# sebasv/lp

Measured on NVIDIA B200. Metric: ipm_iterations_per_s, higher is better.
Workload: dtype f64

## Files before the change

### lp_b200/build.py

```python
from __future__ import annotations

import os
import subprocess
import sys
from concurrent.futures import ThreadPoolExecutor

HERE = os.path.dirname(os.path.abspath(__file__))
CSRC = os.path.join(HERE, "csrc")
LIBDIR = os.path.join(HERE, "_lib")
OBJDIR = os.path.join(LIBDIR, "obj")
LIB = os.path.join(LIBDIR, "liblpb200.so")
SOURCES = ["vec_kernels.cu", "dmma_gemm.cu", "cholesky.cu", "batched.cu", "presolve.cu", "lpb_api.cu"]
NVCC = os.environ.get("NVCC", "/usr/local/cuda/bin/nvcc")
FLAGS = ["-gencode", "arch=compute_100a,code=sm_100a", "-O3", "-std=c++17", "-lineinfo",
         "-Xcompiler", "-fPIC", "-Xcompiler", "-fvisibility=hidden"] + os.environ.get("LPB_EXTRA_NVCC_FLAGS", "").split()


def _deps():
    out = []
    for root in (CSRC, os.path.join(HERE, "..", "include")):
        for f in os.listdir(root):
            if f.endswith((".cu", ".cuh", ".hpp", ".h")):
                out.append(os.path.join(root, f))
    return out


def _stale(target, deps):
    if not os.path.exists(target):
        return True
    t = os.path.getmtime(target)
    return any(os.path.getmtime(d) > t for d in deps)


def build(force: bool = False, verbose: bool = True) -> str:
    os.makedirs(OBJDIR, exist_ok=True)
    deps = _deps()
    srcs = [s for s in SOURCES if os.path.exists(os.path.join(CSRC, s))]

    def compile_one(src):
        obj = os.path.join(OBJDIR, src.replace(".cu", ".o"))
        if force or _stale(obj, deps):
            cmd = [NVCC] + FLAGS + ["-c", os.path.join(CSRC, src), "-o", obj]
            if verbose:
                print(" ".join(cmd), flush=True)
            subprocess.check_call(cmd)
        return obj

    with ThreadPoolExecutor(max_workers=4) as ex:
        objs = list(ex.map(compile_one, srcs))
    if force or _stale(LIB, objs):
        cmd = [NVCC, "-shared", "-o", LIB] + objs + ["-lnccl", "-Xlinker", "-rpath=/usr/local/cuda/lib64"]
        if verbose:
            print(" ".join(cmd), flush=True)
        subprocess.check_call(cmd)
    return LIB


if __name__ == "__main__":
    print(build(force="--force" in sys.argv))
```

### lp_b200/csrc/common.cuh

```cuda
#pragma once
#include <cuda_runtime.h>
#include <cstdint>
#include <cstdio>
#include <cstring>
#include <mutex>

#include "../../include/lpb200.h"

namespace lpb {

void set_last_error(const char* fmt, ...);
const char* get_last_error();

#define LPB_CUDA(call)                                                                         \
  do {                                                                                         \
    cudaError_t e__ = (call);                                                                  \
    if (e__ != cudaSuccess) {                                                                  \
      ::lpb::set_last_error("%s:%d %s -> %s", __FILE__, __LINE__, #call, cudaGetErrorString(e__)); \
      return LPB_ERR_CUDA;                                                                     \
    }                                                                                          \
  } while (0)

#define LPB_TRY(call)              \
  do {                             \
    int rc__ = (call);             \
    if (rc__ != LPB_OK) return rc__; \
  } while (0)

constexpr int kNumSMs = 148;

constexpr int kMaxDevices = 64;
struct PerDeviceOnce {
  std::mutex mu;
  bool done[kMaxDevices] = {};
  template <class F>
  int run(F&& f) {
    int dev = 0;
    LPB_CUDA(cudaGetDevice(&dev));
    if (dev < 0 || dev >= kMaxDevices) return f(dev);
    std::lock_guard<std::mutex> g(mu);
    if (done[dev]) return LPB_OK;
    const int rc = f(dev);
    if (rc == LPB_OK) done[dev] = true;
    return rc;
  }
};

inline int64_t round_up(int64_t v, int64_t a) { return (v + a - 1) / a * a; }
inline int64_t ceil_div(int64_t a, int64_t b) { return (a + b - 1) / b; }

constexpr int kMaxRedVals = 8;
constexpr int kMaxRedBlocks = 1024;
enum RedOp : int { kRedSum = 0, kRedMin = 1 };

struct LaunchCtx {
  cudaStream_t stream = nullptr;
  int64_t launches = 0;
  double* red_partials = nullptr;
  double* red_out = nullptr;
  double* red_host = nullptr;
  unsigned long long* fault_dev = nullptr;
  double* gemv_partials = nullptr;
  int64_t gemv_partials_cap = 0;
  double* chol_ws = nullptr;
  int64_t chol_ws_cap = 0;
  int64_t ws_m = -1;
  int64_t linv_valid_m = -1;
  const double* linv_mat = nullptr;
  bool linv_full = false;
  int solve_epoch = 0;
  int solve_impl = 0;
  int sync_each_launch = 0;
  int syrk_flush_blocks = 32;
  int syrk_tail_split = 1;
  double* syrk_ws = nullptr;
  int64_t syrk_ws_cap = 0;
  int syrk_chain = 0;
  int potf2_impl = 0;
  int trsm_impl = 0, update_impl = 0;
  int solve_grid_cap = 0;
  void* nccl_comm = nullptr;
  int rank = 0, world = 1;
  int potrf_dist = 2;
  double* panel_buf = nullptr;
  int64_t panel_buf_cap = 0;
  int potrf_lookahead = 1;
  cudaStream_t side_stream = nullptr;
  cudaEvent_t ev_col[2] = {nullptr, nullptr}, ev_pan[2] = {nullptr, nullptr};
  bool launch_on_side = false;
  cudaEvent_t ev_dist[4] = {nullptr, nullptr, nullptr, nullptr};
  double* panel_slot[2] = {nullptr, nullptr};
  int64_t panel_slot_cap = 0;
  static constexpr int kMaxPeers = 8;
  double* ring_base = nullptr;
  int64_t ring_slot_doubles = 0;
  int ring_slots = 0;
  double* peer_base[kMaxPeers] = {};
  bool peer_mapped = false;
  bool peer_ready = false;
  uint32_t dist_epoch = 0;
  int update_grid_cap = 0;
  int* info_dev = nullptr;
  int* info_host = nullptr;
};

}
```

### lp_b200/csrc/kernels.hpp

```cpp
#pragma once
#include "common.cuh"

namespace lpb {

struct RedSpec {
  int nvals = 0;
  int nblocks[kMaxRedVals] = {0};
  int op[kMaxRedVals] = {0};
};
int reduce_finalize(LaunchCtx& lc, const RedSpec& spec);
int fetch_scalars(LaunchCtx& lc, int nvals);

int k_fill(LaunchCtx& lc, double* p, int64_t n, double v);
int k_copy(LaunchCtx& lc, double* dst, const double* src, int64_t n);
int k_dinv(LaunchCtx& lc, int64_t n, const double* x, const double* z, double* dinv);

int k_rhat(LaunchCtx& lc, int64_t n, int mode, double eta, double gm, double a2, double s, const double* x,
           const double* z, const double* rD, const double* dx, const double* dz, double* xs, double* r1);

int k_assemble_delta_n(LaunchCtx& lc, int64_t n, double d_tau, const double* u, const double* p, const double* xs,
                       const double* x, const double* z, double* dx, double* dz, int val_base, int* nblocks);
int k_assemble_delta_m(LaunchCtx& lc, int64_t m, double d_tau, const double* v, const double* q, double* dy);
int k_step(LaunchCtx& lc, int64_t n, double alpha, int clamp, double* x, const double* dx);
int k_extract_x(LaunchCtx& lc, int64_t n, double tau, const double* x, const double* c, double* xo, int val,
                int* nblocks);

int k_resid_p(LaunchCtx& lc, int64_t m, double tau, const double* b, const double* t, const double* y, double* rP,
              int val_base, int* nblocks);
int k_sym_fwd_rhs(LaunchCtx& lc, int64_t m, double eta, const double* rP, const double* b, const double* t0,
                  const double* t1, double* rhs0, double* rhs1, int with_pq);
int k_refine_rhs(LaunchCtx& lc, int64_t m, double eta, const double* rP, const double* b, const double* au,
                 const double* ap, double* rho0, double* rho1, int with_pq);
int k_add_inplace(LaunchCtx& lc, int64_t count, const double* x, double* y);
int k_dots_m(LaunchCtx& lc, int64_t m, const double* b, const double* v, const double* q, int with_pq, int val_base,
             int* nblocks);

int k_gemv_n(LaunchCtx& lc, int64_t m, int64_t n, const double* A, int64_t lda, const double* dinv, const double* w0,
             const double* w1, double* t0, double* t1, int nrhs);
int k_gemv_t_partials(LaunchCtx& lc, int64_t m, int64_t n, const double* A, int64_t lda, const double* v0,
                      const double* v1, int nrhs, int* nchunks);
struct TailCols {
  int64_t nd;
  const int* col_row;
  const double* col_val;
  const double* v0;
  const double* v1;
};
int k_gemv_t_raw(LaunchCtx& lc, int64_t n, int nchunks, int nrhs, double* out0, double* out1);
int k_resid_d(LaunchCtx& lc, int64_t n, int nchunks, double tau, const double* c, const double* z, const double* x,
              double* rD, int val_base, int* nblocks, const TailCols* tail = nullptr);
int k_sym_back(LaunchCtx& lc, int64_t n, int nchunks, int with_pq, const double* dinv, const double* r1,
               const double* c, double* u, double* p, int val_base, int* nblocks, const TailCols* tail = nullptr);

int k_syrk_dmma(LaunchCtx& lc, int64_t m, int64_t n, const double* A, int64_t lda, const double* d, double* Cmat,
                int64_t ldc);
int k_trailing_update_dmma(LaunchCtx& lc, int64_t m, double* Mat, int64_t ldm, int64_t k0, int64_t kb);
int k_trailing_update_part(LaunchCtx& lc, int64_t m, double* Mat, int64_t ldm, int64_t k0, int64_t kb, int tile0,
                           int single_col, int own_mod, int own_rem, const double* packed = nullptr,
                           int64_t packed_rows = 0);
int k_trsm_dmma(LaunchCtx& lc, int64_t m, double* Mat, int64_t ldm, int64_t k0, const double* Linv);
int k_dmma_peak(LaunchCtx& lc, double seconds, double* tflops);
int k_syrk_simple(LaunchCtx& lc, int64_t m, int64_t n, const double* A, int64_t lda, const double* d, double* Cmat,
                  int64_t ldc);
int k_trailing_update_simple(LaunchCtx& lc, int64_t m, double* Mat, int64_t ldm, int64_t k0, int64_t kb);

int k_potrf(LaunchCtx& lc, int64_t m, double* Mat, int64_t ldm, int syrk_impl);
int k_potrf_dist_reserve(LaunchCtx& lc, int64_t m);
int k_peer_export(LaunchCtx& lc, int64_t m, unsigned char* handle_out, int* state_out);
int k_peer_import(LaunchCtx& lc, const unsigned char* handles, int world);
void k_peer_release(LaunchCtx& lc);
void k_peer_abandon(LaunchCtx& lc);
void k_peer_free_process();
int k_potrs(LaunchCtx& lc, int64_t m, const double* L, int64_t ldm, double* B, int nrhs, bool use_linv);

int k_fill_normal(LaunchCtx& lc, double* A, int64_t rows, int64_t cols, int64_t lda, int64_t row0, int64_t col0,
                  uint64_t seed);
int k_fill_vec(LaunchCtx& lc, double* v, int64_t count, int64_t idx0, uint64_t seed, int kind, double lo, double hi,
               int64_t neg_below);
int k_slack_identity(LaunchCtx& lc, double* A, int64_t rows, int64_t cols, int64_t lda, int64_t col0, int64_t n0);
int k_add_vec(LaunchCtx& lc, double* out, const double* a, const double* b, int64_t count, int64_t count_b);
int k_col_structure(LaunchCtx& lc, const double* A, int64_t m, int64_t n, int64_t lda, int* nnz, int* row, double* val);
int k_diag_add(LaunchCtx& lc, int64_t m, double* M, int64_t ldm, const int* col, const double* val, const double* dinv);
int k_diag_shift(LaunchCtx& lc, int64_t m, double* M, int64_t ldm, double delta);
int k_slack_add(LaunchCtx& lc, int64_t m, const int* col, const double* val, const double* dinv, const double* w0,
                const double* w1, double* t0, double* t1, int nrhs);
int64_t tri_packed_doubles(int64_t m);
int k_tri_pack(LaunchCtx& lc, double* M, int64_t ldm, int64_t m, double* buf, bool pack);
int k_diff(LaunchCtx& lc, const double* a, const double* b, int64_t rows, int64_t cols, int64_t ld, int lower_only,
           unsigned long long* out_dev3);
int k_checksum(LaunchCtx& lc, const double* v, int64_t rows, int64_t cols, int64_t ld, int lower_only,
               unsigned long long* out_dev);

}
```

### lp_b200/csrc/lpb_api.cu

```cuda
#include <nccl.h>

#include <algorithm>
#include <chrono>
#include <cmath>
#include <cstdlib>
#include <mutex>
#include <new>
#include <string>
#include <vector>

#include "ipm_driver.hpp"
#include "kernels.hpp"

namespace lpb {
int64_t gemv_t_partials_doubles(int64_t m, int64_t n);
int batched_launch(int64_t batch, int m, int n, const double* dA, const double* db, const double* dc,
                   const lpb_options& o, double* dx, double* dfun, int64_t* dit, int32_t* dst, cudaStream_t stream);
int solve_many_check_shape(int64_t m, int64_t n);
int solve_many_launch(int64_t batch, int m, int n, const double* dA, const double* db, const double* dc,
                      const lpb_options& o, double* dx, double* dfun, int64_t* dit, int32_t* dst, cudaStream_t stream);
}

using namespace lpb;

// ... 201 lines not shown
    *nchunks = 0;
    if (c->n_dense > 0) LPB_TRY(k_gemv_t_partials(c->lc, c->m, c->n_dense, c->A, c->lda, v0, v1, nrhs, nchunks));
    *tail = TailCols{c->n_dense, c->col_row, c->col_val, v0, v1};
    return LPB_OK;
  }

  int blind_start() {
    PhaseTimer tm(c, PH_VEC);
    LPB_TRY(k_fill(c->lc, c->x, c->n, 1.0));
    LPB_TRY(k_fill(c->lc, c->z, c->n, 1.0));
    LPB_TRY(k_fill(c->lc, c->y, c->m, 0.0));
    c->have_pq = false;
    return LPB_OK;
  }

  int residuals(double tau, double kappa, lpb_residual_scalars* o) {
    (void)kappa;
    RedSpec spec;
    spec.nvals = 5;
    int nb_n = 0, nb_m = 0, nchunks = 0;
    {
      PhaseTimer tm(c, PH_SWEEP);
      LPB_TRY(sweep_n(nullptr, c->x, nullptr, c->t, nullptr, 1));
    }
    LPB_TRY(allreduce(c, c->t, c->m, ncclSum));
    LPB_TRY(check_replicated(c, "A x after the all-reduce", c->t, 1, c->m, c->m, 0));
    LPB_TRY(check_replicated(c, "y", c->y, 1, c->m, c->m, 0));
    {
      PhaseTimer tm(c, PH_SWEEP);
      LPB_TRY(k_resid_p(c->lc, c->m, tau, c->b, c->t, c->y, c->rP, 3, &nb_m));
      TailCols tail;
      LPB_TRY(sweep_t(c->y, nullptr, 1, &nchunks, &tail));
      LPB_TRY(k_resid_d(c->lc, c->n, nchunks, tau, c->c, c->z, c->x, c->rD, 0, &nb_n, &tail));
    }
    spec.nblocks[0] = spec.nblocks[1] = spec.nblocks[2] = nb_n;
    spec.nblocks[3] = spec.nblocks[4] = nb_m;
    LPB_TRY(finish_scalars(c, spec, 3, ncclSum));
    const double* h = c->lc.red_host;
    o->nrm_rd = std::sqrt(h[0]);
    o->cx = h[1];
    o->xz = h[2];
    o->nrm_rp = std::sqrt(h[3]);
    o->by = h[4];
    return LPB_OK;
  }

  int form_normal_matrix() {
    {
      PhaseTimer tm(c, PH_SYRK);
      if (c->n_dense <= 0)
        LPB_CUDA(cudaMemsetAsync(c->M, 0, sizeof(double) * (size_t)(c->m * c->ldm), c->lc.stream));
      else if (c->syrk_impl == 1)
        LPB_TRY(k_syrk_simple(c->lc, c->m, c->n_dense, c->A, c->lda, c->dinv, c->M, c->ldm));
      else
        LPB_TRY(k_syrk_dmma(c->lc, c->m, c->n_dense, c->A, c->lda, c->dinv, c->M, c->ldm));
      if (c->n_singleton > 0) LPB_TRY(k_diag_add(c->lc, c->m, c->M, c->ldm, c->sgl_col, c->sgl_val, c->dinv));
      c->prof.syrk_launches++;
      c->prof.syrk_cols = c->n_dense;
    }
    if (c->world > 1 && c->packed_allreduce) {
      const int64_t cnt = tri_packed_doubles(c->m);
      if (!c->tri_buf) {
        LPB_TRY(dev_alloc(c, &c->tri_buf, cnt));
        LPB_CUDA(cudaMemsetAsync(c->tri_buf, 0, sizeof(double) * (size_t)cnt, c->lc.stream));
      }
      {
        PhaseTimer tm(c, PH_COMM);
        LPB_TRY(k_tri_pack(c->lc, c->M, c->ldm, c->m, c->tri_buf, true));
      }
      LPB_TRY(allreduce(c, c->tri_buf, cnt, ncclSum));
      {
        PhaseTimer tm(c, PH_COMM);
        LPB_TRY(k_tri_pack(c->lc, c->M, c->ldm, c->m, c->tri_buf, false));
      }
    } else {
      LPB_TRY(allreduce(c, c->M, c->m * c->ldm, ncclSum));
    }
    return check_replicated(c, "M after the all-reduce", c->M, c->m, c->m, c->ldm, 1);
  }

  int factor_normal_matrix(int* info_out) {
    const size_t mbytes = sizeof(double) * (size_t)(c->m * c->ldm);
    if (c->potrf_verify) {
      if (!c->vfy1) {
        LPB_TRY(dev_alloc(c, &c->vfy1, c->m * c->ldm));
        LPB_TRY(dev_alloc(c, &c->vfy2, c->m * c->ldm));
      }
      LPB_CUDA(cudaMemcpyAsync(c->vfy1, c->M, mbytes, cudaMemcpyDeviceToDevice, c->lc.stream));
    }
    {
      PhaseTimer tm(c, PH_POTRF);
      LPB_TRY(k_potrf(c->lc, c->m, c->M, c->ldm, c->syrk_impl));
      c->prof.potrf_launches++;
    }
    if (c->potrf_verify) {
      LPB_CUDA(cudaMemcpyAsync(c->vfy2, c->M, mbytes, cudaMemcpyDeviceToDevice, c->lc.stream));
      LPB_CUDA(cudaMemcpyAsync(c->M, c->vfy1, mbytes, cudaMemcpyDeviceToDevice, c->lc.stream));
      const int saved = c->lc.sync_each_launch;
      if (c->potrf_verify == 2) c->lc.sync_each_launch = 1;
      LPB_TRY(k_potrf(c->lc, c->m, c->M, c->ldm, c->syrk_impl));
      c->lc.sync_each_launch = saved;
      unsigned long long* d3 = nullptr;
      LPB_CUDA(cudaMalloc(reinterpret_cast<void**>(&d3), 3 * sizeof(unsigned long long)));
      LPB_TRY(k_diff(c->lc, c->M, c->vfy2, c->m, c->m, c->ldm, 1, d3));
      unsigned long long h3[3];
      LPB_CUDA(cudaMemcpyAsync(h3, d3, sizeof(h3), cudaMemcpyDeviceToHost, c->lc.stream));
// ... 312 lines not shown
    --nd;
  }
  if (n - nd < 16) return LPB_OK;
  for (int64_t j = nd; j < n; ++j)
    if (nnz[j] != 1) h_int[(size_t)(n + j)] = -1;
  LPB_CUDA(cudaMemcpyAsync(c->sgl_col, col_of_row.data(), sizeof(int) * (size_t)m, cudaMemcpyHostToDevice, c->lc.stream));
  LPB_CUDA(cudaMemcpyAsync(c->sgl_val, sq.data(), sizeof(double) * (size_t)m, cudaMemcpyHostToDevice, c->lc.stream));
  LPB_CUDA(cudaMemcpyAsync(c->col_row, row, sizeof(int) * (size_t)n, cudaMemcpyHostToDevice, c->lc.stream));
  LPB_CUDA(cudaMemcpyAsync(c->col_val, h_val.data(), sizeof(double) * (size_t)n, cudaMemcpyHostToDevice, c->lc.stream));
  LPB_CUDA(cudaStreamSynchronize(c->lc.stream));
  c->n_dense = nd;
  c->n_singleton = nsgl;
  return LPB_OK;
}

int upload_problem(lpb_ctx* c, const double* A, int64_t lda, const double* b, const double* cc, double c0, int mem) {
  if (!A || !b || !cc || lda < c->n) {
    set_last_error("set_problem: null pointer or lda < n");
    return LPB_ERR_BAD_ARGUMENT;
  }
  const cudaMemcpyKind kind = mem == LPB_MEM_DEVICE ? cudaMemcpyDeviceToDevice : cudaMemcpyHostToDevice;
  if (lda == c->lda && lda == c->n)
    LPB_CUDA(cudaMemcpyAsync(c->A, A, sizeof(double) * (size_t)(c->m * c->lda), kind, c->lc.stream));
  else
    LPB_CUDA(cudaMemcpy2DAsync(c->A, sizeof(double) * c->lda, A, sizeof(double) * lda, sizeof(double) * c->n, c->m,
                               kind, c->lc.stream));
  LPB_CUDA(cudaMemcpyAsync(c->b, b, sizeof(double) * c->m, kind, c->lc.stream));
  LPB_CUDA(cudaMemcpyAsync(c->c, cc, sizeof(double) * c->n, kind, c->lc.stream));
  if (std::getenv("LPB_TIME_CREATE")) {
    const auto t0 = std::chrono::steady_clock::now();
    LPB_CUDA(cudaStreamSynchronize(c->lc.stream));
    const double ms = std::chrono::duration<double, std::milli>(std::chrono::steady_clock::now() - t0).count();
    std::fprintf(stderr, "[upload] copies drained in %.1f ms after issue (%.1f GB/s)\n", ms,
                 8.0 * c->m * c->n / (ms * 1e-3) / 1e9);
  }
  LPB_CUDA(cudaStreamSynchronize(c->lc.stream));
  c->c0 = c0;
  c->has_problem = true;
  c->have_pq = false;
  return analyze_structure(c);
}

void ctx_free(lpb_ctx* c) {
  if (!c) return;
  if (c->lc.stream) cudaStreamSynchronize(c->lc.stream);
  for (auto& r : c->recs) {
    cudaEventDestroy(r.a);
    cudaEventDestroy(r.b);
  }
  for (auto e : c->ev_free) cudaEventDestroy(e);
  for (void* p : c->allocs) cudaFree(p);
  if (c->lc.chol_ws) cudaFree(c->lc.chol_ws);
  if (c->lc.syrk_ws) cudaFree(c->lc.syrk_ws);
  if (c->lc.panel_buf) cudaFree(c->lc.panel_buf);
  k_peer_release(c->lc);
  for (int i = 0; i < 2; ++i)
    if (c->lc.panel_slot[i]) cudaFree(c->lc.panel_slot[i]);
  for (int e = 0; e < 4; ++e)
    if (c->lc.ev_dist[e]) cudaEventDestroy(c->lc.ev_dist[e]);
  if (c->lc.side_stream) {
    cudaStreamSynchronize(c->lc.side_stream);
    for (int e = 0; e < 2; ++e) {
      if (c->lc.ev_col[e]) cudaEventDestroy(c->lc.ev_col[e]);
      if (c->lc.ev_pan[e]) cudaEventDestroy(c->lc.ev_pan[e]);
    }
    cudaStreamDestroy(c->lc.side_stream);
  }
  if (c->lc.red_host) cudaFreeHost(c->lc.red_host);
  if (c->lc.info_host) cudaFreeHost(c->lc.info_host);
  if (c->chk_host) cudaFreeHost(c->chk_host);
  if (c->own_stream && c->lc.stream) cudaStreamDestroy(c->lc.stream);
  if (c->comm) {
    std::lock_guard<std::mutex> g(g_comm_mu);
    if (c->comm == g_comm.comm && g_comm.refs > 0) --g_comm.refs;
  }
  delete c;
}

int need_problem(lpb_ctx* c) {
  if (!c || !c->has_problem) {
    set_last_error("context has no problem attached");
    return LPB_ERR_BAD_ARGUMENT;
  }
  return LPB_OK;
}

using BatchedLaunch = int (*)(int64_t, int, int, const double*, const double*, const double*, const lpb_options&, double*,
                              double*, int64_t*, int32_t*, cudaStream_t);

int run_batched(BatchedLaunch launch, int64_t batch, int64_t m, int64_t n, const double* A, const double* b, const double* c,
                const lpb_options& o, double* x_out, double* fun, int64_t* iterations, int32_t* status, int mem,
                cudaStream_t st) {
  if (mem == LPB_MEM_DEVICE) {
    LPB_TRY(launch(batch, (int)m, (int)n, A, b, c, o, x_out, fun, iterations, status, st));
    LPB_CUDA(cudaStreamSynchronize(st));
    return LPB_OK;
  }
  const size_t sA = sizeof(double) * (size_t)(batch * m * n), sb = sizeof(double) * (size_t)(batch * m),
               sc = sizeof(double) * (size_t)(batch * n), s8 = sizeof(double) * (size_t)batch,
               s4 = sizeof(int32_t) * (size_t)batch;
  auto up = [](size_t v) { return (v + 255) & ~(size_t)255; };
  const size_t need = up(sA) + up(sb) + 2 * up(sc) + 2 * up(s8) + up(s4);
  if (g_batched_ws_cap < need) {
    if (g_batched_ws) cudaFree(g_batched_ws);
    g_batched_ws = nullptr;
    g_batched_ws_cap = 0;
// ... 459 lines not shown
  return d.extract_x(tau, x_out, fun);
}

int lpb_solve(lpb_ctx* c, const lpb_options* opts, double* x_out, double* fun, int64_t* iterations) {
  LPB_TRY(need_problem(c));
  lpb_options o;
  if (opts)
    o = *opts;
  else
    options_default(&o);
  LPB_TRY(lpb_options_validate(&o));
  profile_reset(c);
  const int64_t launches0 = c->lc.launches;
  cudaEvent_t e0 = nullptr, e1 = nullptr;
  if (c->profile) {
    LPB_CUDA(cudaEventCreate(&e0));
    LPB_CUDA(cudaEventCreate(&e1));
    LPB_CUDA(cudaEventRecord(e0, c->lc.stream));
  }
  CudaDev dev{c};
  int rc = solve_normal_form(dev, o, c->n_global, c->c0, &c->last);
  if (iterations) *iterations = c->last.iterations;
  if (rc == LPB_OK || rc == LPB_ERR_ITERATION_LIMIT_EXCEEDED) {
    const int rc2 = dev.extract_x(c->last.tau, x_out, fun);
    if (rc2 != LPB_OK) rc = rc2;
  }
  if (c->profile) {
    cudaEventRecord(e1, c->lc.stream);
    cudaEventSynchronize(e1);
    float f = 0.f;
    cudaEventElapsedTime(&f, e0, e1);
    profile_collect(c);
    c->prof.total_ms = f;
    cudaEventDestroy(e0);
    cudaEventDestroy(e1);
  }
  c->prof.launches = c->lc.launches - launches0;
  c->prof.iterations = c->last.iterations;
  return rc;
}

int64_t lpb_trace(lpb_ctx* c, double* rows, int64_t max_rows) {
  if (!c || !rows) return 0;
  int64_t k = 0;
  for (; k < (int64_t)c->last.trace.size() && k < max_rows; ++k)
    std::memcpy(rows + k * LPB_TRACE_COLS, c->last.trace[k].v, sizeof(double) * LPB_TRACE_COLS);
  return k;
}

int lpb_k_syrk_adat(lpb_ctx* c, int64_t m, int64_t n, const double* dA, int64_t lda, const double* d_d, double* dM,
                    int64_t ldm) {
  if (!c || !dA || !dM) return LPB_ERR_BAD_ARGUMENT;
  int rc = c->syrk_impl == 1 ? k_syrk_simple(c->lc, m, n, dA, lda, d_d, dM, ldm)
                             : k_syrk_dmma(c->lc, m, n, dA, lda, d_d, dM, ldm);
  if (rc != LPB_OK) return rc;
  LPB_CUDA(cudaStreamSynchronize(c->lc.stream));
  return LPB_OK;
}

int lpb_k_potrf(lpb_ctx* c, int64_t m, double* dM, int64_t ldm, int32_t* info_host) {
  if (!c || !dM) return LPB_ERR_BAD_ARGUMENT;
  LPB_TRY(k_potrf(c->lc, m, dM, ldm, c->syrk_impl));
  LPB_CUDA(cudaMemcpyAsync(c->lc.info_host, c->lc.info_dev, sizeof(int), cudaMemcpyDeviceToHost, c->lc.stream));
  LPB_CUDA(cudaStreamSynchronize(c->lc.stream));
  if (info_host) *info_host = *c->lc.info_host;
  return LPB_OK;
}

int lpb_k_potrs(lpb_ctx* c, int64_t m, const double* dL, int64_t ldm, double* dB, int64_t nrhs) {
  if (!c || !dL || !dB) return LPB_ERR_BAD_ARGUMENT;
  LPB_TRY(k_potrs(c->lc, m, dL, ldm, dB, (int)nrhs, c->syrk_impl == 0));
  return fetch_scalars(c->lc, 0);
}

int lpb_k_gemv_n(lpb_ctx* c, int64_t m, int64_t n, const double* dA, int64_t lda, const double* d_w, double* d_out) {
  if (!c || !dA || !d_w || !d_out) return LPB_ERR_BAD_ARGUMENT;
  LPB_TRY(k_gemv_n(c->lc, m, n, dA, lda, nullptr, d_w, nullptr, d_out, nullptr, 1));
  LPB_CUDA(cudaStreamSynchronize(c->lc.stream));
  return LPB_OK;
}

int lpb_k_gemv_t(lpb_ctx* c, int64_t m, int64_t n, const double* dA, int64_t lda, const double* d_v, double* d_out) {
  if (!c || !dA || !d_v || !d_out) return LPB_ERR_BAD_ARGUMENT;
  if (gemv_t_partials_doubles(m, n) > c->lc.gemv_partials_cap) {
    set_last_error("gemv_t: context work buffers were sized for a smaller problem");
    return LPB_ERR_BAD_ARGUMENT;
  }
  int nchunks = 0;
  LPB_TRY(k_gemv_t_partials(c->lc, m, n, dA, lda, d_v, nullptr, 1, &nchunks));
  LPB_TRY(k_gemv_t_raw(c->lc, n, nchunks, 1, d_out, nullptr));
  LPB_CUDA(cudaStreamSynchronize(c->lc.stream));
  return LPB_OK;
}

int lpb_solve_batched(int64_t batch, int64_t m, int64_t n, const double* A, const double* b, const double* c,
                      const lpb_options* opts, double* x_out, double* fun, int64_t* iterations, int32_t* status,
                      int mem, void* stream) {
  lpb_options o;
  LPB_TRY(batched_args("solve_batched", batch, m, n, A, b, c, opts, x_out, fun, iterations, status, &o));
  LPB_TRY(check_device());
  return run_batched(batched_launch, batch, m, n, A, b, c, o, x_out, fun, iterations, status, mem,
                     static_cast<cudaStream_t>(stream));
}

int lpb_solve_many(int64_t batch, int64_t m, int64_t n, const double* A, const double* b, const double* c,
                   const lpb_options* opts, double* x_out, double* fun, int64_t* iterations, int32_t* status, int mem,
                   void* stream) {
// ... 3 lines not shown
  LPB_TRY(check_device());
  return run_batched(solve_many_launch, batch, m, n, A, b, c, o, x_out, fun, iterations, status, mem,
                     static_cast<cudaStream_t>(stream));
}

int lpb_release_workspaces(void) {
  if (g_batched_ws) cudaFree(g_batched_ws);
  g_batched_ws = nullptr;
  g_batched_ws_cap = 0;
  if (g_batched_copy_stream) cudaStreamDestroy(g_batched_copy_stream);
  g_batched_copy_stream = nullptr;
  for (int q = 0; q < 4; ++q) {
    if (g_batched_ev[q]) cudaEventDestroy(g_batched_ev[q]);
    g_batched_ev[q] = nullptr;
  }
  return LPB_OK;
}

int lpb_get_profile(lpb_ctx* c, lpb_profile* out) {
  if (!c || !out) return LPB_ERR_BAD_ARGUMENT;
  *out = c->prof;
  return LPB_OK;
}

int64_t lpb_launch_count(lpb_ctx* c) { return c ? c->lc.launches : 0; }

int lpb_measure_dmma_peak(lpb_ctx* c, double seconds, double* tflops_out) {
  if (!c || !tflops_out) return LPB_ERR_BAD_ARGUMENT;
  return k_dmma_peak(c->lc, seconds, tflops_out);
}

int lpb_set_option(lpb_ctx* c, const char* key, int64_t value) {
  if (!c || !key) return LPB_ERR_BAD_ARGUMENT;
  const std::string k(key);
  if (k == "syrk_impl") {
    if (value != 0 && value != 1) return LPB_ERR_BAD_ARGUMENT;
    c->syrk_impl = (int)value;
    return LPB_OK;
  }
  if (k == "solve_impl") {
    if (value < 0 || value > 3) return LPB_ERR_BAD_ARGUMENT;
    c->lc.solve_impl = (int)value;
    return LPB_OK;
  }
  if (k == "trsm_impl" || k == "update_impl") {
    if (value < 0 || value > 6) return LPB_ERR_BAD_ARGUMENT;
    (k == "trsm_impl" ? c->lc.trsm_impl : c->lc.update_impl) = (int)value;
    return LPB_OK;
  }
  if (k == "syrk_tail_split") {
    c->lc.syrk_tail_split = value != 0;
    return LPB_OK;
  }
  if (k == "syrk_chain") {
    c->lc.syrk_chain = value != 0;
    return LPB_OK;
  }
  if (k == "peer_panels") {
    if (value > 0 && !c->lc.peer_mapped) return LPB_ERR_BAD_ARGUMENT;
    if (value < 0)
      k_peer_abandon(c->lc);
    else
      c->lc.peer_ready = value != 0;
    return LPB_OK;
  }
  if (k == "syrk_flush_blocks") {
    if (value < 32 || value > (1 << 20) || (value & (value - 1))) return LPB_ERR_BAD_ARGUMENT;
    c->lc.syrk_flush_blocks = (int)value;
    return LPB_OK;
  }
  if (k == "potf2_impl") {
    if (value < 0 || value > 1) return LPB_ERR_BAD_ARGUMENT;
    c->lc.potf2_impl = (int)value;
    if (value == 1) c->lc.trsm_impl = 1;
    return LPB_OK;
  }
  if (k == "solve_grid_cap") {
    if (value < 0) return LPB_ERR_BAD_ARGUMENT;
    c->lc.solve_grid_cap = (int)value;
    return LPB_OK;
  }
  if (k == "refine") {
    if (value < 0 || value > 4) return LPB_ERR_BAD_ARGUMENT;
    c->refine = (int)value;
    return LPB_OK;
  }
  if (k == "refine_max") {
    if (value < 0 || value > 8) return LPB_ERR_BAD_ARGUMENT;
    c->refine_max = (int)value;
    return LPB_OK;
  }
  if (k == "regularize") {
    c->regularize = value != 0;
    return LPB_OK;
  }
  if (k == "structure") {
    c->use_structure = value != 0;
    return c->has_problem ? analyze_structure(c) : LPB_OK;
  }
  if (k == "potrf_lookahead") {
    c->lc.potrf_lookahead = value != 0;
    return LPB_OK;
  }
  if (k == "packed_allreduce") {
    c->packed_allreduce = value != 0;
    return LPB_OK;
// ... 28 lines not shown
```

Before: 3.994.

## Emulate FP64 SYRK with int8 tensor-core GEMMs via CRT (Ozaki scheme)

```diff
diff --git a/lp_b200/build.py b/lp_b200/build.py
--- a/lp_b200/build.py
+++ b/lp_b200/build.py
@@ -10,7 +10,7 @@
 LIBDIR = os.path.join(HERE, "_lib")
 OBJDIR = os.path.join(LIBDIR, "obj")
 LIB = os.path.join(LIBDIR, "liblpb200.so")
-SOURCES = ["vec_kernels.cu", "dmma_gemm.cu", "cholesky.cu", "batched.cu", "presolve.cu", "lpb_api.cu"]
+SOURCES = ["vec_kernels.cu", "dmma_gemm.cu", "syrk_i8.cu", "cholesky.cu", "batched.cu", "presolve.cu", "lpb_api.cu"]
 NVCC = os.environ.get("NVCC", "/usr/local/cuda/bin/nvcc")
 FLAGS = ["-gencode", "arch=compute_100a,code=sm_100a", "-O3", "-std=c++17", "-lineinfo",
          "-Xcompiler", "-fPIC", "-Xcompiler", "-fvisibility=hidden"] + os.environ.get("LPB_EXTRA_NVCC_FLAGS", "").split()
diff --git a/lp_b200/csrc/common.cuh b/lp_b200/csrc/common.cuh
--- a/lp_b200/csrc/common.cuh
+++ b/lp_b200/csrc/common.cuh
@@ -76,6 +76,18 @@
   double* syrk_ws = nullptr;
   int64_t syrk_ws_cap = 0;
   int syrk_chain = 0;
+  int syrk_emu = 2;
+  int64_t syrk_emu_cap = int64_t{16} << 30;
+  int8_t* i8_ops = nullptr;
+  int64_t i8_ops_cap = 0;
+  int8_t* i8_res = nullptr;
+  int64_t i8_res_cap = 0;
+  int* i8_ex = nullptr;
+  int64_t i8_ex_cap = 0;
+  int2* i8_tiles = nullptr;
+  int64_t i8_tiles_cap = 0;
+  int64_t i8_tiles_m = -1;
+  int i8_ntiles = 0;
   int potf2_impl = 0;
   int trsm_impl = 0, update_impl = 0;
   int solve_grid_cap = 0;
diff --git a/lp_b200/csrc/kernels.hpp b/lp_b200/csrc/kernels.hpp
--- a/lp_b200/csrc/kernels.hpp
+++ b/lp_b200/csrc/kernels.hpp
@@ -64,6 +64,13 @@
                   int64_t ldc);
 int k_trailing_update_simple(LaunchCtx& lc, int64_t m, double* Mat, int64_t ldm, int64_t k0, int64_t kb);
 
+int k_syrk_i8(LaunchCtx& lc, int64_t m, int64_t n, const double* A, int64_t lda, const double* d, double* Cmat,
+              int64_t ldc);
+int64_t syrk_i8_chunk(const LaunchCtx& lc, int64_t m, int64_t n);
+constexpr int64_t kSyrkEmuMinM = 2048, kSyrkEmuMinN = 2048;
+bool syrk_i8_selected(const LaunchCtx& lc, int64_t m, int64_t n);
+void syrk_i8_free(LaunchCtx& lc);
+
 int k_potrf(LaunchCtx& lc, int64_t m, double* Mat, int64_t ldm, int syrk_impl);
 int k_potrf_dist_reserve(LaunchCtx& lc, int64_t m);
 int k_peer_export(LaunchCtx& lc, int64_t m, unsigned char* handle_out, int* state_out);
diff --git a/lp_b200/csrc/lpb_api.cu b/lp_b200/csrc/lpb_api.cu
--- a/lp_b200/csrc/lpb_api.cu
+++ b/lp_b200/csrc/lpb_api.cu
@@ -277,6 +277,8 @@
         LPB_CUDA(cudaMemsetAsync(c->M, 0, sizeof(double) * (size_t)(c->m * c->ldm), c->lc.stream));
       else if (c->syrk_impl == 1)
         LPB_TRY(k_syrk_simple(c->lc, c->m, c->n_dense, c->A, c->lda, c->dinv, c->M, c->ldm));
+      else if (syrk_i8_selected(c->lc, c->m, c->n_dense))
+        LPB_TRY(k_syrk_i8(c->lc, c->m, c->n_dense, c->A, c->lda, c->dinv, c->M, c->ldm));
       else
         LPB_TRY(k_syrk_dmma(c->lc, c->m, c->n_dense, c->A, c->lda, c->dinv, c->M, c->ldm));
       if (c->n_singleton > 0) LPB_TRY(k_diag_add(c->lc, c->m, c->M, c->ldm, c->sgl_col, c->sgl_val, c->dinv));
@@ -695,6 +697,7 @@
   for (void* p : c->allocs) cudaFree(p);
   if (c->lc.chol_ws) cudaFree(c->lc.chol_ws);
   if (c->lc.syrk_ws) cudaFree(c->lc.syrk_ws);
+  syrk_i8_free(c->lc);
   if (c->lc.panel_buf) cudaFree(c->lc.panel_buf);
   k_peer_release(c->lc);
   for (int i = 0; i < 2; ++i)
@@ -1260,7 +1263,8 @@
                     int64_t ldm) {
   if (!c || !dA || !dM) return LPB_ERR_BAD_ARGUMENT;
   int rc = c->syrk_impl == 1 ? k_syrk_simple(c->lc, m, n, dA, lda, d_d, dM, ldm)
-                             : k_syrk_dmma(c->lc, m, n, dA, lda, d_d, dM, ldm);
+           : c->lc.syrk_emu == 1 && syrk_i8_selected(c->lc, m, n) ? k_syrk_i8(c->lc, m, n, dA, lda, d_d, dM, ldm)
+                                                                  : k_syrk_dmma(c->lc, m, n, dA, lda, d_d, dM, ldm);
   if (rc != LPB_OK) return rc;
   LPB_CUDA(cudaStreamSynchronize(c->lc.stream));
   return LPB_OK;
@@ -1370,6 +1374,16 @@
     c->lc.syrk_tail_split = value != 0;
     return LPB_OK;
   }
+  if (k == "syrk_emu") {
+    if (value < 0 || value > 2) return LPB_ERR_BAD_ARGUMENT;
+    c->lc.syrk_emu = (int)value;
+    return LPB_OK;
+  }
+  if (k == "syrk_emu_cap_mb") {
+    if (value < 1 || value > (int64_t{1} << 30)) return LPB_ERR_BAD_ARGUMENT;
+    c->lc.syrk_emu_cap = value << 20;
+    return LPB_OK;
+  }
   if (k == "syrk_chain") {
     c->lc.syrk_chain = value != 0;
     return LPB_OK;
diff --git a/lp_b200/csrc/syrk_i8.cu b/lp_b200/csrc/syrk_i8.cu
--- /dev/null
+++ b/lp_b200/csrc/syrk_i8.cu
@@ -0,0 +1,558 @@
+#include <cuda.h>
+
+#include <algorithm>
+#include <vector>
+
+#include "kernels.hpp"
+
+namespace lpb {
+
+namespace {
+
+constexpr int kMods = 16;
+__host__ __device__ constexpr int modulus(int l) {
+  return l == 0 ? 256 : l == 1 ? 255 : l == 2 ? 253 : l == 3 ? 251 : l == 4 ? 247 : l == 5 ? 241 : l == 6 ? 239
+       : l == 7 ? 233 : l == 8 ? 229 : l == 9 ? 227 : l == 10 ? 223 : l == 11 ? 217 : l == 12 ? 211 : l == 13 ? 199
+       : l == 14 ? 197 : 193;
+}
+constexpr int kPBits = 126;
+constexpr int64_t kMaxChunk = 32768;
+
+constexpr int BM = 128, BN = 256, BKB = 128, kStages = 4;
+constexpr int kBand = 12;
+constexpr uint32_t kABytes = BM * BKB, kBBytes = BN * BKB, kStageBytes = kABytes + kBBytes;
+constexpr uint32_t kBarOff = kStages * kStageBytes;
+constexpr uint32_t kSmem = kBarOff + 256 + 1024;
+constexpr int kThreads = 192;
+constexpr int kSplitThreads = 256;
+
+int beta_for(int64_t k) {
+  int b = 0;
+  while ((int64_t{1} << b) < k) ++b;
+  return (kPBits - 2 - b) / 2;
+}
+
+__device__ __forceinline__ uint32_t smem_u32(const void* p) { return (uint32_t)__cvta_generic_to_shared(p); }
+__device__ __forceinline__ void mbar_init(uint32_t bar, uint32_t c) {
+  asm volatile("mbarrier.init.shared::cta.b64 [%0], %1;" ::"r"(bar), "r"(c) : "memory");
+}
+__device__ __forceinline__ void mbar_expect_tx(uint32_t bar, uint32_t b) {
+  asm volatile("mbarrier.arrive.expect_tx.shared::cta.b64 _, [%0], %1;" ::"r"(bar), "r"(b) : "memory");
+}
+__device__ __forceinline__ void mbar_arrive(uint32_t bar) {
+  asm volatile("mbarrier.arrive.shared::cta.b64 _, [%0];" ::"r"(bar) : "memory");
+}
+__device__ __forceinline__ uint32_t mbar_try_wait(uint32_t bar, uint32_t ph) {
+  uint32_t ok;
+  asm volatile(
+      "{\n\t.reg .pred p;\n\tmbarrier.try_wait.parity.shared::cta.b64 p, [%1], %2;\n\tselp.u32 %0, 1, 0, p;\n\t}"
+      : "=r"(ok)
+      : "r"(bar), "r"(ph)
+      : "memory");
+  return ok;
+}
+__device__ __forceinline__ void mbar_wait(uint32_t bar, uint32_t ph) {
+  if (mbar_try_wait(bar, ph)) return;
+  const long long t0 = clock64();
+  while (!mbar_try_wait(bar, ph))
+    if (clock64() - t0 > 8000000000ll) __trap();
+}
+__device__ __forceinline__ void tma_load_2d(uint32_t dst, const CUtensorMap* tm, int c0, int c1, uint32_t bar) {
+  asm volatile(
+      "cp.async.bulk.tensor.2d.shared::cluster.global.mbarrier::complete_tx::bytes [%0], [%1, {%2, %3}], [%4];" ::"r"(
+          dst),
+      "l"((uint64_t)tm), "r"(c0), "r"(c1), "r"(bar)
+      : "memory");
+}
+__device__ __forceinline__ void tc_fence_before() { asm volatile("tcgen05.fence::before_thread_sync;" ::: "memory"); }
+__device__ __forceinline__ void tc_fence_after() { asm volatile("tcgen05.fence::after_thread_sync;" ::: "memory"); }
+__device__ __forceinline__ uint64_t sdesc(uint32_t a) {
+  return (uint64_t)((a & 0x3FFFFu) >> 4) | ((uint64_t)1 << 16) | ((uint64_t)(1024 >> 4) << 32) | ((uint64_t)1 << 46) |
+         ((uint64_t)2 << 61);
+}
+__device__ __forceinline__ void mma_i8(uint32_t d, uint64_t a, uint64_t b, uint32_t idesc, uint32_t acc) {
+  asm volatile(
+      "{\n\t.reg .pred p;\n\tsetp.ne.b32 p, %4, 0;\n\ttcgen05.mma.cta_group::1.kind::i8 [%0], %1, %2, %3, p;\n\t}" ::"r"(d),
+      "l"(a), "l"(b), "r"(idesc), "r"(acc)
+      : "memory");
+}
+__device__ __forceinline__ void mma_commit(uint32_t bar) {
+  asm volatile("tcgen05.commit.cta_group::1.mbarrier::arrive::one.shared::cluster.b64 [%0];" ::"r"(bar) : "memory");
+}
+#define LPB_R8(i) \
+  "=r"(v[i]), "=r"(v[i + 1]), "=r"(v[i + 2]), "=r"(v[i + 3]), "=r"(v[i + 4]), "=r"(v[i + 5]), "=r"(v[i + 6]), "=r"(v[i + 7])
+__device__ __forceinline__ void tmem_ld32(uint32_t taddr, int (&v)[32]) {
+  asm volatile(
+      "tcgen05.ld.sync.aligned.32x32b.x32.b32 {%0,%1,%2,%3,%4,%5,%6,%7,%8,%9,%10,%11,%12,%13,%14,%15,"
+      "%16,%17,%18,%19,%20,%21,%22,%23,%24,%25,%26,%27,%28,%29,%30,%31}, [%32];"
+      : LPB_R8(0), LPB_R8(8), LPB_R8(16), LPB_R8(24)
+      : "r"(taddr));
+  asm volatile("tcgen05.wait::ld.sync.aligned;" ::: "memory");
+}
+#undef LPB_R8
+
+template <int P>
+__device__ __forceinline__ int sym_mod(int v) {
+  int r = v % P;
+  if (r > (P - 1) / 2) r -= P;
+  else if (r < -(P / 2)) r += P;
+  return r;
+}
+
+__device__ __forceinline__ int dexp(double x) {
+  int e;
+  frexp(x, &e);
+  return e;
+}
+__device__ __forceinline__ void split_d(double d, double* s1, double* s2) {
+  if (!(d > 0.0)) {
+    *s1 = 1.0;
+    *s2 = d;
+    return;
+  }
+  const int p = (dexp(d) - 1) >> 1;
+  *s1 = ldexp(1.0, p);
+  *s2 = ldexp(d, -p);
+}
+__device__ __forceinline__ void residues(double x, int (&r)[kMods]) {
+  const double kMagic = 6755399441055744.0;
+#pragma unroll
+  for (int l = 0; l < kMods; ++l) {
+    constexpr double one = 1.0;
+    const double p = (double)modulus(l);
+    const double q = fma(x, one / p, kMagic) - kMagic;
+    const double rr = fma(-q, p, x) + kMagic;
+    int v = __double2loint(rr);
+    if (v > (modulus(l) - 1) / 2) v -= modulus(l);
+    else if (v < -(modulus(l) / 2)) v += modulus(l);
+    r[l] = v;
+  }
+}
+
+__global__ void __launch_bounds__(kSplitThreads)
+i8_split_kernel(const double* __restrict__ A, int64_t lda, const double* __restrict__ d, int64_t k0, int kc, int kpad,
+                int m_pad, int beta, int8_t* __restrict__ ops, int* __restrict__ ex) {
+  const int i = blockIdx.x;
+  const double* a = A + (int64_t)i * lda + k0;
+  double mx1 = 0.0, mx2 = 0.0;
+  for (int k = threadIdx.x; k < kc; k += kSplitThreads) {
+    double s1, s2;
+    split_d(d ? d[k0 + k] : 1.0, &s1, &s2);
+    const double v = a[k];
+    mx1 = fmax(mx1, fabs(v * s1));
+    mx2 = fmax(mx2, fabs(v * s2));
+  }
+  __shared__ double red[2][kSplitThreads / 32];
+#pragma unroll
+  for (int o = 16; o; o >>= 1) {
+    mx1 = fmax(mx1, __shfl_xor_sync(0xffffffffu, mx1, o));
+    mx2 = fmax(mx2, __shfl_xor_sync(0xffffffffu, mx2, o));
+  }
+  if ((threadIdx.x & 31) == 0) {
+    red[0][threadIdx.x >> 5] = mx1;
+    red[1][threadIdx.x >> 5] = mx2;
+  }
+  __syncthreads();
+  mx1 = mx2 = 0.0;
+#pragma unroll
+  for (int w = 0; w < kSplitThreads / 32; ++w) {
+    mx1 = fmax(mx1, red[0][w]);
+    mx2 = fmax(mx2, red[1][w]);
+  }
+  const int e1 = mx1 > 0.0 ? dexp(mx1) : 0, e2 = mx2 > 0.0 ? dexp(mx2) : 0;
+  if (threadIdx.x == 0) {
+    ex[i] = e1;
+    ex[m_pad + i] = e2;
+  }
+  const double t1 = ldexp(1.0, beta - e1), t2 = ldexp(1.0, beta - e2);
+  const int64_t plane = (int64_t)m_pad * kpad;
+  int8_t* o1 = ops + (int64_t)i * kpad;
+  int8_t* o2 = o1 + kMods * plane;
+  for (int k = 4 * threadIdx.x; k < kpad; k += 4 * kSplitThreads) {
+    uint32_t w1[kMods], w2[kMods];
+#pragma unroll
+    for (int l = 0; l < kMods; ++l) w1[l] = w2[l] = 0;
+#pragma unroll
+    for (int j = 0; j < 4; ++j) {
+      double x1 = 0.0, x2 = 0.0;
+      if (k + j < kc) {
+        double s1, s2;
+        split_d(d ? d[k0 + k + j] : 1.0, &s1, &s2);
+        const double v = a[k + j];
+        x1 = rint((v * s1) * t1);
+        x2 = rint((v * s2) * t2);
+      }
+      int r[kMods];
+      residues(x1, r);
+#pragma unroll
+      for (int l = 0; l < kMods; ++l) w1[l] |= (uint32_t)(r[l] & 0xff) << (8 * j);
+      residues(x2, r);
+#pragma unroll
+      for (int l = 0; l < kMods; ++l) w2[l] |= (uint32_t)(r[l] & 0xff) << (8 * j);
+    }
+#pragma unroll
+    for (int l = 0; l < kMods; ++l) {
+      *reinterpret_cast<uint32_t*>(o1 + l * plane + k) = w1[l];
+      *reinterpret_cast<uint32_t*>(o2 + l * plane + k) = w2[l];
+    }
+  }
+}
+
+__global__ void __launch_bounds__(kThreads, 1)
+i8_syrk_kernel(const __grid_constant__ CUtensorMap tmA, const __grid_constant__ CUtensorMap tmB, int8_t* __restrict__ res,
+               int m_pad, int nkb, const int2* __restrict__ tiles, int ntiles) {
+  extern __shared__ __align__(1024) uint8_t smem_raw[];
+  const uint32_t base = (smem_u32(smem_raw) + 1023u) & ~1023u;
+  const uint32_t sA = base, sB = base + kStages * kABytes, bars = base + kBarOff;
+  const uint32_t full = bars, empty = bars + 8 * kStages, tfull = bars + 16 * kStages, tempty = tfull + 16,
+                 tslot = tempty + 16;
+  const int warp = threadIdx.x >> 5, lane = threadIdx.x & 31;
+  const int nitems = kMods * ntiles;
+  if (threadIdx.x == 0) {
+    for (int s = 0; s < kStages; ++s) {
+      mbar_init(full + 8 * s, 1);
+      mbar_init(empty + 8 * s, 1);
+    }
+    for (int a = 0; a < 2; ++a) {
+      mbar_init(tfull + 8 * a, 1);
+      mbar_init(tempty + 8 * a, 4);
+    }
+    asm volatile("fence.mbarrier_init.release.cluster;" ::: "memory");
+  }
+  if (warp == 1) {
+    asm volatile("tcgen05.alloc.cta_group::1.sync.aligned.shared::cta.b32 [%0], %1;" ::"r"(tslot), "r"(2 * BN)
+                 : "memory");
+    asm volatile("tcgen05.relinquish_alloc_permit.cta_group::1.sync.aligned;" ::: "memory");
+  }
+  tc_fence_before();
+  __syncthreads();
+  tc_fence_after();
+  uint32_t tmem;
+  asm volatile("ld.shared.u32 %0, [%1];" : "=r"(tmem) : "r"(tslot) : "memory");
+
+  if (warp == 0) {
+    if (lane == 0) {
+      int s = 0;
+      uint32_t ph = 0;
+      for (int I = blockIdx.x; I < nitems; I += gridDim.x) {
+        const int l = I / ntiles;
+        const int2 tl = tiles[I - l * ntiles];
+        const int ra = l * m_pad + tl.x * BM, rb = l * m_pad + tl.y * BN;
+        for (int kb = 0; kb < nkb; ++kb) {
+          mbar_wait(empty + 8 * s, ph ^ 1u);
+          mbar_expect_tx(full + 8 * s, kStageBytes);
+          tma_load_2d(sA + s * kABytes, &tmA, kb * BKB, ra, full + 8 * s);
+          tma_load_2d(sB + s * kBBytes, &tmB, kb * BKB, rb, full + 8 * s);
+          if (++s == kStages) {
+            s = 0;
+            ph ^= 1u;
+          }
+        }
+      }
+    }
+  } else if (warp == 1) {
+    if (lane == 0) {
+      const uint32_t idesc =
+          (2u << 4) | (1u << 7) | (1u << 10) | ((uint32_t)(BN >> 3) << 17) | ((uint32_t)(BM >> 4) << 24);
+      int s = 0;
+      uint32_t ph = 0;
+      int it = 0;
+      for (int I = blockIdx.x; I < nitems; I += gridDim.x, ++it) {
+        const int acc = it & 1;
+        mbar_wait(tempty + 8 * acc, (((uint32_t)it >> 1) & 1u) ^ 1u);
+        tc_fence_after();
+        const uint32_t dt = tmem + acc * BN;
+        for (int kb = 0; kb < nkb; ++kb) {
+          mbar_wait(full + 8 * s, ph);
+          tc_fence_after();
+#pragma unroll
+          for (int kk = 0; kk < BKB / 32; ++kk)
+            mma_i8(dt, sdesc(sA + s * kABytes + kk * 32), sdesc(sB + s * kBBytes + kk * 32), idesc, (kb | kk) != 0);
+          mma_commit(empty + 8 * s);
+          if (++s == kStages) {
+            s = 0;
+            ph ^= 1u;
+          }
+        }
+        mma_commit(tfull + 8 * acc);
+      }
+    }
+  } else {
+    const int q = warp & 3;
+    int it = 0;
+    for (int I = blockIdx.x; I < nitems; I += gridDim.x, ++it) {
+      const int acc = it & 1;
+      const int l = I / ntiles;
+      const int2 tl = tiles[I - l * ntiles];
+      mbar_wait(tfull + 8 * acc, ((uint32_t)it >> 1) & 1u);
+      tc_fence_after();
+      const int row = tl.x * BM + q * 32 + lane;
+      int8_t* crow = res + ((int64_t)l * m_pad + row) * m_pad + (int64_t)tl.y * BN;
+      const uint32_t taddr = tmem + ((uint32_t)(q * 32) << 16) + acc * BN;
+#pragma unroll 1
+      for (int c = 0; c < BN; c += 32) {
+        int v[32];
+        tmem_ld32(taddr + c, v);
+        uint32_t w[8];
+#define LPB_MODCASE(L)                                                                        \
+  case L:                                                                                     \
+    _Pragma("unroll") for (int x = 0; x < 8; ++x) {                                           \
+      w[x] = 0;                                                                               \
+      _Pragma("unroll") for (int y = 0; y < 4; ++y) w[x] |=                                   \
+          ((uint32_t)(sym_mod<modulus(L)>(v[4 * x + y]) & 0xff)) << (8 * y);                  \
+    }                                                                                         \
+    break;
+        switch (l) {
+          LPB_MODCASE(0) LPB_MODCASE(1) LPB_MODCASE(2) LPB_MODCASE(3) LPB_MODCASE(4) LPB_MODCASE(5) LPB_MODCASE(6)
+          LPB_MODCASE(7) LPB_MODCASE(8) LPB_MODCASE(9) LPB_MODCASE(10) LPB_MODCASE(11) LPB_MODCASE(12)
+          LPB_MODCASE(13) LPB_MODCASE(14) default : LPB_MODCASE(15)
+        }
+#undef LPB_MODCASE
+        int4* dst = reinterpret_cast<int4*>(crow + c);
+        dst[0] = make_int4(w[0], w[1], w[2], w[3]);
+        dst[1] = make_int4(w[4], w[5], w[6], w[7]);
+      }
+      tc_fence_before();
+      __syncwarp();
+      if (lane == 0) mbar_arrive(tempty + 8 * acc);
+    }
+  }
+  __syncthreads();
+  if (warp == 1) {
+    __syncwarp();
+    tc_fence_after();
+    asm volatile("tcgen05.dealloc.cta_group::1.sync.aligned.b32 %0, %1;" ::"r"(tmem), "r"(2 * BN) : "memory");
+  }
+}
+
+struct CrtConst {
+  unsigned long long mlo[kMods], mhi[kMods];
+  int inv[kMods];
+  unsigned long long plo, phi;
+};
+
+__device__ __forceinline__ double crt_value(const int (&r)[kMods], const CrtConst& cc, int scale) {
+  unsigned __int128 x = 0;
+  double qf = 0.0;
+#pragma unroll
+  for (int l = 0; l < kMods; ++l) {
+    int t = (r[l] * cc.inv[l]) % modulus(l);
+    if (t < 0) t += modulus(l);
+    x += (unsigned __int128)(((unsigned __int128)cc.mhi[l] << 64) | cc.mlo[l]) * (unsigned)t;
+    qf += (double)t * (1.0 / modulus(l));
+  }
+  const unsigned long long q = (unsigned long long)rint(qf);
+  x -= (((unsigned __int128)cc.phi << 64) | cc.plo) * q;
+  const bool neg = (__int128)x < 0;
+  unsigned __int128 u = neg ? (unsigned __int128)(-(__int128)x) : x;
+  const unsigned long long hi = (unsigned long long)(u >> 64), lo = (unsigned long long)u;
+  double v;
+  if (hi == 0) {
+    v = __ull2double_rn(lo);
+  } else {
+    const int sh = 64 - __clzll(hi);
+    const unsigned long long top = (unsigned long long)(u >> sh) | ((lo << (64 - sh)) != 0 ? 1ull : 0ull);
+    v = ldexp(__ull2double_rn(top), sh);
+  }
+  v = ldexp(v, scale);
+  return neg ? -v : v;
+}
+
+__global__ void __launch_bounds__(256)
+i8_crt_kernel(const int8_t* __restrict__ res, const int* __restrict__ ex, int m, int m_pad, int beta2, CrtConst cc,
+              double* __restrict__ C, int64_t ldc, int accumulate) {
+  int ti, tj;
+  {
+    const int L = blockIdx.x;
+    int i = (int)((sqrt(8.0 * (double)L + 1.0) - 1.0) * 0.5);
+    while (i * (i + 1) / 2 > L) --i;
+    while ((i + 1) * (i + 2) / 2 <= L) ++i;
+    ti = i;
+    tj = L - i * (i + 1) / 2;
+  }
+  const int64_t plane = (int64_t)m_pad * m_pad;
+  for (int e = threadIdx.x; e < 128 * 16; e += 256) {
+    const int r = ti * 128 + (e >> 4), c0 = tj * 128 + (e & 15) * 8;
+    if (r >= m) continue;
+    uint2 w[kMods];
+#pragma unroll
+    for (int l = 0; l < kMods; ++l) w[l] = *reinterpret_cast<const uint2*>(res + l * plane + (int64_t)r * m_pad + c0);
+    const int er = ex[r];
+#pragma unroll
+    for (int j = 0; j < 8; ++j) {
+      const int c = c0 + j;
+      if (c >= m) break;
+      int rv[kMods];
+#pragma unroll
+      for (int l = 0; l < kMods; ++l) rv[l] = (int)(int8_t)((j < 4 ? w[l].x >> (8 * j) : w[l].y >> (8 * (j - 4))) & 0xff);
+      const double v = crt_value(rv, cc, er + ex[m_pad + c] - beta2);
+      double* dst = C + (int64_t)r * ldc + c;
+      *dst = accumulate ? *dst + v : v;
+    }
+  }
+}
+
+typedef CUresult (*EncodeTiledFn)(CUtensorMap*, CUtensorMapDataType, cuuint32_t, void*, const cuuint64_t*,
+                                  const cuuint64_t*, const cuuint32_t*, const cuuint32_t*, CUtensorMapInterleave,
+                                  CUtensorMapSwizzle, CUtensorMapL2promotion, CUtensorMapFloatOOBfill);
+
+int make_tmap_i8(CUtensorMap* tm, const int8_t* base, uint64_t rows, uint64_t cols, uint32_t box_rows) {
+  static std::mutex mu;
+  static EncodeTiledFn fn = nullptr;
+  std::lock_guard<std::mutex> g(mu);
+  if (!fn) {
+    void* p = nullptr;
+    cudaDriverEntryPointQueryResult q;
+    LPB_CUDA(cudaGetDriverEntryPoint("cuTensorMapEncodeTiled", &p, cudaEnableDefault, &q));
+    if (q != cudaDriverEntryPointSuccess || !p) {
+      set_last_error("cuTensorMapEncodeTiled not available from the driver");
+      return LPB_ERR_CUDA;
+    }
+    fn = reinterpret_cast<EncodeTiledFn>(p);
+  }
+  const cuuint64_t dims[2] = {cols, rows};
+  const cuuint64_t strides[1] = {cols};
+  const cuuint32_t box[2] = {BKB, box_rows};
+  const cuuint32_t es[2] = {1, 1};
+  const CUresult r = fn(tm, CU_TENSOR_MAP_DATA_TYPE_UINT8, 2, const_cast<int8_t*>(base), dims, strides, box, es,
+                        CU_TENSOR_MAP_INTERLEAVE_NONE, CU_TENSOR_MAP_SWIZZLE_128B, CU_TENSOR_MAP_L2_PROMOTION_L2_256B,
+                        CU_TENSOR_MAP_FLOAT_OOB_FILL_NONE);
+  if (r != CUDA_SUCCESS) {
+    set_last_error("cuTensorMapEncodeTiled (int8 planes) failed (%d)", (int)r);
+    return LPB_ERR_CUDA;
+  }
+  return LPB_OK;
+}
+
+CrtConst crt_constants() {
+  using u128 = unsigned __int128;
+  u128 P = 1;
+  for (int l = 0; l < kMods; ++l) P *= (u128)modulus(l);
+  CrtConst cc;
+  for (int l = 0; l < kMods; ++l) {
+    const u128 Ml = P / (u128)modulus(l);
+    cc.mlo[l] = (unsigned long long)Ml;
+    cc.mhi[l] = (unsigned long long)(Ml >> 64);
+    const int mr = (int)(Ml % (u128)modulus(l));
+    int inv = 1;
+    while ((mr * inv) % modulus(l) != 1) ++inv;
+    cc.inv[l] = inv;
+  }
+  cc.plo = (unsigned long long)P;
+  cc.phi = (unsigned long long)(P >> 64);
+  return cc;
+}
+
+std::vector<int2> tile_list(int m) {
+  const int ntr = (int)ceil_div(m, BM);
+  std::vector<int2> t;
+  for (int r0 = 0; r0 < ntr; r0 += kBand) {
+    const int r1 = std::min(ntr, r0 + kBand);
+    for (int c = 0; c <= (r1 - 1) / 2; ++c)
+      for (int r = std::max(r0, 2 * c); r < r1; ++r) t.push_back(make_int2(r, c));
+  }
+  return t;
+}
+
+template <class T>
+int grow(T** p, int64_t* cap, int64_t need) {
+  if (*cap >= need) return LPB_OK;
+  if (*p) LPB_CUDA(cudaFree(*p));
+  *p = nullptr;
+  *cap = 0;
+  void* q = nullptr;
+  LPB_CUDA(cudaMalloc(&q, sizeof(T) * (size_t)need));
+  *p = static_cast<T*>(q);
+  *cap = need;
+  return LPB_OK;
+}
+
+PerDeviceOnce g_attr_once;
+
+}
+
+int64_t syrk_i8_chunk(const LaunchCtx& lc, int64_t m, int64_t n) {
+  const int64_t m_pad = round_up(m, BN);
+  int64_t kc = std::min<int64_t>(round_up(n, BKB), kMaxChunk);
+  const int64_t fit = lc.syrk_emu_cap / (2 * kMods * m_pad) / BKB * BKB;
+  if (fit < kc) kc = fit;
+  return kc;
+}
+
+bool syrk_i8_selected(const LaunchCtx& lc, int64_t m, int64_t n) {
+  if (lc.syrk_emu == 0) return false;
+  if (lc.syrk_chain || lc.syrk_flush_blocks != 32 || !lc.syrk_tail_split) return false;
+  if (syrk_i8_chunk(lc, m, n) < 1024) return false;
+  if (lc.syrk_emu == 1) return true;
+  return m >= kSyrkEmuMinM && n >= kSyrkEmuMinN;
+}
+
+int k_syrk_i8(LaunchCtx& lc, int64_t m, int64_t n, const double* A, int64_t lda, const double* d, double* C,
+              int64_t ldc) {
+  if (m <= 0 || n <= 0) return LPB_OK;
+  if (m > (1 << 20) / 2) {
+    set_last_error("syrk_i8: m too large");
+    return LPB_ERR_BAD_ARGUMENT;
+  }
+  const int64_t kc_max = syrk_i8_chunk(lc, m, n);
+  if (kc_max < BKB) {
+    set_last_error("syrk_i8: the workspace cap (option syrk_emu_cap_mb) holds no K-block");
+    return LPB_ERR_BAD_ARGUMENT;
+  }
+  LPB_TRY(g_attr_once.run([](int) {
+    LPB_CUDA(cudaFuncSetAttribute(i8_syrk_kernel, cudaFuncAttributeMaxDynamicSharedMemorySize, kSmem));
+    return LPB_OK;
+  }));
+  const int m_pad = (int)round_up(m, BN);
+  const int64_t kpad_max = kc_max;
+  LPB_TRY(grow(&lc.i8_ops, &lc.i8_ops_cap, 2 * kMods * (int64_t)m_pad * kpad_max));
+  LPB_TRY(grow(&lc.i8_res, &lc.i8_res_cap, kMods * (int64_t)m_pad * m_pad));
+  LPB_TRY(grow(&lc.i8_ex, &lc.i8_ex_cap, 2 * (int64_t)m_pad));
+  if (lc.i8_tiles_m != m) {
+    const std::vector<int2> tl = tile_list((int)m);
+    LPB_TRY(grow(&lc.i8_tiles, &lc.i8_tiles_cap, (int64_t)tl.size()));
+    LPB_CUDA(cudaMemcpy(lc.i8_tiles, tl.data(), sizeof(int2) * tl.size(), cudaMemcpyHostToDevice));
+    lc.i8_tiles_m = m;
+    lc.i8_ntiles = (int)tl.size();
+  }
+  static const CrtConst cc = crt_constants();
+  for (int64_t k0 = 0; k0 < n; k0 += kc_max) {
+    const int kc = (int)std::min<int64_t>(kc_max, n - k0);
+    const int kpad = (int)round_up(kc, BKB);
+    const int beta = beta_for(kc);
+    if (m < m_pad)
+      LPB_CUDA(cudaMemset2DAsync(lc.i8_ops + m * kpad, (size_t)m_pad * kpad, 0, (size_t)(m_pad - m) * kpad, 2 * kMods,
+                                 lc.stream));
+    i8_split_kernel<<<(unsigned)m, kSplitThreads, 0, lc.stream>>>(A, lda, d, k0, kc, kpad, m_pad, beta, lc.i8_ops,
+                                                                  lc.i8_ex);
+    LPB_CUDA(cudaGetLastError());
+    CUtensorMap tmA, tmB;
+    LPB_TRY(make_tmap_i8(&tmA, lc.i8_ops, (uint64_t)kMods * m_pad, (uint64_t)kpad, BM));
+    LPB_TRY(make_tmap_i8(&tmB, lc.i8_ops + (int64_t)kMods * m_pad * kpad, (uint64_t)kMods * m_pad, (uint64_t)kpad, BN));
+    const int grid = std::min(kNumSMs, kMods * lc.i8_ntiles);
+    i8_syrk_kernel<<<grid, kThreads, kSmem, lc.stream>>>(tmA, tmB, lc.i8_res, m_pad, kpad / BKB, lc.i8_tiles,
+                                                         lc.i8_ntiles);
+    LPB_CUDA(cudaGetLastError());
+    const int ntr = (int)ceil_div(m, 128);
+    i8_crt_kernel<<<(unsigned)(ntr * (ntr + 1) / 2), 256, 0, lc.stream>>>(lc.i8_res, lc.i8_ex, (int)m, m_pad, 2 * beta,
+                                                                          cc, C, ldc, k0 > 0);
+    LPB_CUDA(cudaGetLastError());
+    lc.launches += 3;
+  }
+  return LPB_OK;
+}
+
+void syrk_i8_free(LaunchCtx& lc) {
+  if (lc.i8_ops) cudaFree(lc.i8_ops);
+  if (lc.i8_res) cudaFree(lc.i8_res);
+  if (lc.i8_ex) cudaFree(lc.i8_ex);
+  if (lc.i8_tiles) cudaFree(lc.i8_tiles);
+  lc.i8_ops = nullptr;
+  lc.i8_res = nullptr;
+  lc.i8_ex = nullptr;
+  lc.i8_tiles = nullptr;
+  lc.i8_ops_cap = lc.i8_res_cap = lc.i8_ex_cap = lc.i8_tiles_cap = 0;
+  lc.i8_tiles_m = -1;
+}
+
+}
```

After: 8.023, median of 6. +100.9%, better.
